# mmurooka/SMPLpp

Measured on AMD Instinct MI355X. Metric: SMPL FK evals/s + IK iters/s, batch 1024 frames, 1/2/4/8 MI355X, higher is better.
Workload: dtype f32 (exact operands: every fp32 value as three bf16 pieces = fp32's 24 bits on the bf16 matrix pipe, fp32 accumulate; fp32 VALU skinning)

## Files before the change

smplpp_amd/csrc/common.h:

```cpp
#pragma once

#include <hip/hip_runtime.h>

#include <cstdint>
#include <cstdio>
#include <cstring>
#include <memory>
#include <string>
#include <utility>
#include <vector>

#include "layout.h"

namespace smplpp_hip
{
__host__ __device__ inline int64_t bcol(int64_t v, int x)
{
  return (v / VG) * (3 * VG) + x * VG + (v % VG);
}

__host__ __device__ inline uint16_t bf16_rn_bits(float x)
{
  uint32_t u;
  memcpy(&u, &x, 4);
// ... 163 lines not shown
  int64_t VGPn = 0;
  smplpp_hip::DevPtr<uint8_t> B2h;
  float sB = 1.0f, sG = 1.0f;
  smplpp_hip::DevPtr<int> range_flag;
  smplpp_hip::DevPtr<uint8_t> B3e;
  char form = 'e';
  char form_ik = 'h';
  smplpp_hip::DevPtr<uint8_t> wIdx;
  smplpp_hip::DevPtr<float> wVal;
  smplpp_hip::DevPtr<float> wSum;
  smplpp_hip::DevPtr<float> J0;
  smplpp_hip::DevPtr<float> JS;
  smplpp_hip::DevPtr<float> JSp;
  smplpp_hip::DevPtr<int32_t> parent;
  smplpp_hip::DevPtr<int32_t> lvl;
  int nlev = 0;
  bool chain_fast = false;
  smplpp_hip::DevPtr<int32_t> faces;
  smplpp_hip::DevPtr<int32_t> adjOff;
  smplpp_hip::DevPtr<int32_t> adjFace;
  int madj = smplpp_hip::MAXADJ;
  smplpp_hip::DevPtr<uint16_t> faceRing;
  smplpp_hip::DevPtr<uint8_t> faceMap;
  smplpp_hip::DevPtr<int32_t> anc;
  smplpp_hip::DevPtr<float> Wdense;
  smplpp_hip::DevPtr<float> Pvm;
  smplpp_hip::DevPtr<float> Svm;
  std::vector<int32_t> h_parent, h_faces, h_adjOff, h_adjFace;
  bool profiling = false;
  std::vector<hipEvent_t> prof_events;
  smplpp_hip::Workspace ws;
  smplpp_hip::Arena arena;
  smplpp_hip::StatePtr<smplpp_hip::VjpState> vjp;
  smplpp_hip::StatePtr<smplpp_hip::NormalsVjpState> nvjp;
  char pd_form = 0;
  smplpp_hip::StatePtr<smplpp_hip::PointDistState> pd;
  smplpp_hip::StatePtr<smplpp_hip::MeshPointDistState> mpd;
  smplpp_hip::StatePtr<smplpp_hip::WindingState> wn;
  smplpp_hip::StatePtr<smplpp_hip::SelfPenState> sp;
  int dr_inline = -1;
  smplpp_hip::StatePtr<smplpp_hip::DepthRasterState> dr;
  smplpp_hip::StatePtr<smplpp_hip::SilhouetteState> sil;
  int vo_frames = 0;
  smplpp_hip::StatePtr<smplpp_hip::VertexOffsetsState> vo;
  ~smplpp_model();
};
// ... 1 lines not shown
```

smplpp_amd/csrc/ik.hip:

```cpp
#include "ik_types.h"
#include "ik_eval.h"
#include "ik_solve.h"
#include "ik_proj.h"
#include "vposer_state.h"

#include <algorithm>
#include <chrono>
#include <cstdlib>
#include <type_traits>

using namespace smplpp_hip;

struct smplpp_ik
{
  smplpp_model * m = nullptr;
  smplpp_vposer * vp = nullptr;
  int64_t n = 0, K = 0;
  int64_t frame_base = 0;
  int theta_dim = TD75;
  TaskArrays ta{};
  float *theta = nullptr, *beta = nullptr, *theta25 = nullptr, *vjac = nullptr;
  float *verts = nullptr, *rest = nullptr, *joints = nullptr, *poserot = nullptr, *pts = nullptr;
  double *e = nullptr, *J = nullptr, *Jl = nullptr, *e2 = nullptr, *xout = nullptr;
  int *skip = nullptr, *status = nullptr, *sticky = nullptr, *list_cnt = nullptr, *list_f = nullptr;
// ... 1 lines not shown
  int32_t * roles = nullptr;
  float * list_d = nullptr;
  std::vector<DevPtr<void>> owned;
  bool have_eval = false;
  int64_t last_D = 0;
  hipStream_t side = nullptr;
  hipEvent_t ev_fork = nullptr, ev_join = nullptr;
  bool phi_locked = false;
  bool side_pending = false;
  int * dbg_buf = nullptr;
  unsigned * sig = nullptr;
  unsigned tick_fork = 0, tick_join = 0, tick_done = 0;
  bool use_flags = false;
  double last_enqueue_us = 0.0;
  bool latent_split = false;
  bool latent_split_default = false;
  bool exact = false;
  StatePtr<VPoserJxWork> jxw;
  bool jac_ahead = false;
  bool dbg_sync = false, overlap_ok = true;
  int dbg_stop = 0;
  int64_t scan_blocks = 1536;
  int scan_form = -1;
  float * vbuf[2] = {nullptr, nullptr};
  int vcur = 0;
  Arena arena;
  ~smplpp_ik()
  {
    (void)hipSetDevice(m->device);
    if(side) (void)hipStreamSynchronize(side);
    if(ev_fork) (void)hipEventDestroy(ev_fork);
    if(ev_join) (void)hipEventDestroy(ev_join);
    if(side) (void)hipStreamDestroy(side);
  }
};

enum Fill { AS_ALLOCATED, ZERO_BYTES, VALUE, DEFAULT_NORMAL };

template<class T>
static hipError_t dalloc(smplpp_ik * s, T *& p, size_t count, Fill fill, float v = 0.0f)
{
  DevPtr<T> d;
  hipError_t e = dev_alloc(d, count);
  p = d.get();
  if(e != hipSuccess) return e;
  s->owned.emplace_back(std::move(d));
// ... 69 lines not shown
  if(m->V > 65535) return fail(SMPLPP_ERR_INVALID, "smplpp_ik_create: at most 65535 vertices are supported (ring tables hold 16-bit ids)");
  if(!m->faceRing || !m->faceMap || !m->anc) return fail(SMPLPP_ERR_INVALID, "smplpp_ik_create: the model carries no ring tables");
  std::vector<int32_t> roles;
  if(const char * why = eval_roles(m->h_parent, EVAL_NT, roles)) return fail(SMPLPP_ERR_INVALID, why);
  if(K > PROJ_MAXK) return fail(SMPLPP_ERR_INVALID, "smplpp_ik_create: at most 48 tasks per frame are supported");
  if(TD75 + 2 * K + NB > MAXD)
    return fail(SMPLPP_ERR_INVALID, "smplpp_ik_create: too many tasks for the in-LDS solver (75 + 2K + 10 must be <= 181)");
  HIP_TRY(hipSetDevice(m->device));
  std::unique_ptr<smplpp_ik> s(new smplpp_ik());
  s->m = m;
  s->vp = vposer;
  s->n = n;
  s->K = K;
  s->theta_dim = vposer ? TD44 : TD75;
  {
    const char * e;
    s->dbg_sync = getenv("SMPLPP_DEBUG_SYNC") != nullptr;
    if((e = getenv("SMPLPP_IK_DBG_STOP"))) s->dbg_stop = atoi(e);
    if((e = getenv("SMPLPP_IK_OVERLAP"))) s->overlap_ok = e[0] != '0';
    if(s->dbg_sync) s->overlap_ok = false;
    s->scan_blocks = default_scan_blocks(n, K, m->F);
    if((e = getenv("SMPLPP_SCAN_BLOCKS"))) s->scan_blocks = atoll(e);
    if((e = getenv("SMPLPP_SCAN_FORM"))) s->scan_form = atoi(e);
    s->latent_split = vposer != nullptr && n <= 128 && s->dbg_stop == 0;
    if((e = getenv("SMPLPP_IK_LATENT_SPLIT"))) s->latent_split = vposer != nullptr && e[0] != '0' && s->dbg_stop == 0;
  }
  const size_t nk = (size_t)n * K;
  const size_t Dmax = TD75 + 2 * K + NB;
  const size_t nV3 = (size_t)n * m->V * 3;
  smplpp_ik * const p = s.get();
  HIP_TRY(dalloc(p, p->ta.face, nk, ZERO_BYTES));
  HIP_TRY(dalloc(p, p->ta.vw, nk * 3, VALUE, 1.0f / 3.0f));
  HIP_TRY(dalloc(p, p->ta.tang, nk * 6, VALUE, 0.0f));
  HIP_TRY(dalloc(p, p->ta.tpos, nk * 3, VALUE, 0.0f));
  HIP_TRY(dalloc(p, p->ta.tnrm, nk * 3, DEFAULT_NORMAL));
  HIP_TRY(dalloc(p, p->ta.posw, nk, VALUE, 1.0f));
  HIP_TRY(dalloc(p, p->ta.nrmw, nk, VALUE, 1.0f));
  HIP_TRY(dalloc(p, p->ta.philim, nk, VALUE, 0.04f));
  HIP_TRY(dalloc(p, p->ta.noff, nk, VALUE, 0.0f));
  HIP_TRY(dalloc(p, p->ta.apos, nk * 3, AS_ALLOCATED));
  HIP_TRY(dalloc(p, p->ta.anrm, nk * 3, AS_ALLOCATED));
  HIP_TRY(dalloc(p, p->ta.hint, nk, AS_ALLOCATED));
  HIP_TRY(dalloc(p, p->ta.roww, nk * 2, AS_ALLOCATED));
  HIP_TRY(dalloc(p, p->theta, (size_t)n * p->theta_dim, ZERO_BYTES));
  HIP_TRY(dalloc(p, p->beta, (size_t)n * NB, ZERO_BYTES));
  HIP_TRY(dalloc(p, p->theta25, (size_t)n * 75, ZERO_BYTES));
// ... 336 lines not shown
                                               solve_form<false, 3>()};
  return forms;
}

static int ik_enqueue_solve(smplpp_ik * s, const SolveCall & c)
{
  {
    TraceRange tr_solve("solve IK");
    const SolveForm * f = solve_forms();
    while(f->dual_only != c.p.dual_only || f->ntr != c.p.ntr) f++;
    f->launch(s, c);
  }
  HIP_TRY(hipGetLastError());
  return SMPLPP_OK;
}

template<int KPR, int NBT>
static void scan_launch(smplpp_ik * s, int chunks, const float * qpts, const float * hint, hipStream_t pst)
{
  proj_scan_kernel<KPR, NBT><<<dim3((unsigned)(s->n * chunks)), dim3(256), 0, pst>>>(view_of(s->m), s->ta, s->verts, qpts, hint, s->m->F, (int)s->K, chunks,
                                                                                    s->skip, s->list_cnt, s->list_d, s->list_f, s->dbg_stop);
}

static int ik_enqueue_reproject(smplpp_ik * s, const SidePlan & sp, int it, const SeqHook * last, hipStream_t st)
{
  smplpp_model * m = s->m;
  const int K = (int)s->K;
  const bool dbg = s->dbg_sync, beside = sp.beside;
  TraceRange tr_proj("project point");
  const float * qpts = beside ? s->ta.apos : s->pts;
  hipStream_t pst = st;
  if(beside)
  {
    if(s->use_flags)
      HIP_TRY(hipStreamWaitValue32(s->side, s->sig, s->tick_fork, hipStreamWaitValueGte, 0xffffffffu));
    else
      HIP_TRY(hipStreamWaitEvent(s->side, s->ev_fork, 0));
    pst = s->side;
  }
  const ScanPlan sc = scan_plan(s->n, K, m->F, s->scan_blocks, s->scan_form);
  const float * hint = beside ? s->ta.hint : nullptr;
  if(sc.nbt3) scan_launch<0, 3>(s, sc.chunks, qpts, hint, pst);
  else if(sc.kpr == 0) scan_launch<0, CP_BATCH>(s, sc.chunks, qpts, hint, pst);
  else if(sc.kpr == 2) scan_launch<2, CP_BATCH>(s, sc.chunks, qpts, hint, pst);
  else scan_launch<4, CP_BATCH>(s, sc.chunks, qpts, hint, pst);
  HIP_TRY(hipGetLastError());
  int *& dbg_buf = s->dbg_buf;
  if(dbg && !dbg_buf) HIP_TRY(dalloc(s, dbg_buf, 8, AS_ALLOCATED));
  if(dbg) HIP_TRY(hipMemsetAsync(dbg_buf, 0, sizeof(int) * 8, st));
  const int fsplit = frame_split(s->n, K);
  if(sp.go) s->tick_join++;
  hipExtLaunchKernelGGL(proj_finish_kernel, dim3((unsigned)(s->n * fsplit)), dim3(256), 0, pst, nullptr,
                        (beside && !s->use_flags) ? s->ev_join : nullptr, 0,
                        view_of(m), s->ta, (const float *)s->verts, qpts, m->F, K, (const int *)s->skip, s->list_cnt, s->list_d,
                        s->list_f, dbg ? dbg_buf : (int *)nullptr, fsplit, sp.join_flag ? s->sig + 32 : (unsigned *)nullptr,
                        sp.join_flag ? s->sig + 48 : (unsigned *)nullptr, s->tick_join, last ? last->next_tpos : (const float *)nullptr,
                        last ? last->next_valid : (const uint8_t *)nullptr, last ? last->shared : 0);
  HIP_TRY(hipGetLastError());
  if(sp.ahead)
  {
    HIP_TRY(hipStreamWaitValue32(s->side, s->sig + 64, s->tick_done, hipStreamWaitValueGte, 0xffffffffu));
    int rc = vposer_forward_device(s->vp, s->n, s->theta + 6, TD44, nullptr, 75, s->vjac, s->side, s->frame_base, false, s->sig + 32,
                                   s->sig + 48, s->tick_join);
    if(rc) return rc;
    s->jac_ahead = true;
  }
  if(beside) s->side_pending = true;
  if(dbg)
  {
    int h[8];
    HIP_TRY(hipMemcpy(h, dbg_buf, sizeof(h), hipMemcpyDeviceToHost));
    fprintf(stderr, "[smplpp dbg] it %d: project lists: tasks %d, empty %d, overflow %d, nan %d, max cnt %d\n", it, h[0], h[1], h[2], h[3], h[4]);
  }
  return SMPLPP_OK;
}

static int ik_iterate_enqueue(smplpp_ik * s, int iters, int enable_qp, int optimize_beta_from, int64_t min_valid, hipStream_t st,
                              const SeqHook * hook = nullptr, bool more_follows = false)
{
  int rc = SMPLPP_OK;
  const int K = (int)s->K;
  static PerDeviceOnce once_solve[SOLVE_FORMS];
  for(int i = 0; i < SOLVE_FORMS; i++) HIP_TRY(lds_opt_in(once_solve[i], s->m->device, solve_forms()[i].kfn, (int)SOLVE_LDS_MAX));
  if(s->use_flags && (s->tick_fork > 0x7fff0000u || s->tick_join > 0x7fff0000u || s->tick_done > 0x7fff0000u))
  {
    HIP_TRY(hipStreamSynchronize(st));
    HIP_TRY(hipStreamSynchronize(s->side));
    HIP_TRY(hipMemset(s->sig, 0, sizeof(unsigned) * 128));
    s->tick_fork = s->tick_join = s->tick_done = 0;
  }
  auto dbg_sync = [&](int it, const char * tag) -> int {
    if(!s->dbg_sync) return SMPLPP_OK;
    fprintf(stderr, "[smplpp dbg] it %d: %s ...\n", it, tag);
    HIP_TRY(hipStreamSynchronize(st));
    fprintf(stderr, "[smplpp dbg] it %d: %s done\n", it, tag);
// ... 174 lines not shown
```

smplpp_amd/csrc/ik_plan.h:

```cpp
#pragma once

#include <algorithm>
#include <cstddef>
#include <vector>

#include "layout.h"

namespace smplpp_hip
{
constexpr int TD75 = SMPLPP_THETA_DIM;
constexpr int TD44 = SMPLPP_LATENT_POSE_DIM;
constexpr int IK_MAXK = 48;
constexpr size_t SOLVE_LDS_MAX = 160 * 1024 - 1536;
constexpr int MAXD = TD75 + 2 * IK_MAXK + NB;

struct IterFlags
{
  int opt_beta, phi_live;
};
inline IterFlags iter_flags(int optimize_beta_from, int it)
{
  const int on = (optimize_beta_from >= 0 && it >= optimize_beta_from) ? 1 : 0;
  return {on, optimize_beta_from >= 0 ? on : 1};
}
// ... 37 lines not shown

inline int64_t default_scan_blocks(int64_t n, int64_t K, int64_t F)
{
  if(n >= 512 && K <= 8 && (F + 767) / 768 <= 32) return n * ((F + 767) / 768);
  return (n >= 256 && n < 512) ? 2 * n : 1536;
}

struct ScanPlan
{
  int chunks;
  int kpr;
  bool nbt3;
};
inline ScanPlan scan_plan(int64_t n, int K, int64_t F, int64_t scan_blocks, int scan_form)
{
  int chunks = (int)(scan_blocks / n);
  chunks = chunks < 1 ? 1 : (chunks > 32 ? 32 : chunks);
  const bool small_chunk = (F + chunks - 1) / chunks <= 3 * 256;
  const bool many = scan_form < 0 ? (n >= 512 && small_chunk) : scan_form == 0;
  const int kpr = (K > 8 || many) ? 0 : (K <= 4 ? 2 : 4);
  return {chunks, kpr, kpr == 0 && small_chunk};
}

inline int frame_split(int64_t n, int K)
{
  const int split = n < 256 ? (int)(256 / n) : 1;
  return std::max(1, std::min(split, K));
}

struct SidePlan
{
  bool beside;
  bool go;
  bool ahead;
  bool join_flag;
};
inline SidePlan side_plan(bool overlap_ok, bool phi_free, bool use_flags, bool latent_split, bool opt_beta, bool another_follows)
{
  SidePlan p;
  p.beside = overlap_ok && !phi_free;
  p.go = p.beside && use_flags;
  p.ahead = latent_split && p.go && !opt_beta && another_follows;
  p.join_flag = p.go && !p.ahead;
  return p;
}

// ... 25 lines not shown
```

smplpp_amd/csrc/ik_proj.h:

```cpp
#pragma once
#include "ik_types.h"

namespace smplpp_hip
{
constexpr int PROJ_LIST = 512;
constexpr int PROJ_MAXK = IK_MAXK;

typedef float f32x2 __attribute__((ext_vector_type(2)));

template<int KPR, int NBT = CP_BATCH>
__global__ __launch_bounds__(256) void proj_scan_kernel(ModelView mv, TaskArrays ta, const float * __restrict__ verts_all,
                                                         const float * __restrict__ pts, const float * __restrict__ hint, int64_t F,
                                                         int K, int chunks, const int * __restrict__ skip, int * __restrict__ list_cnt,
                                                         float * __restrict__ list_d, int * __restrict__ list_f, int dbg_stop)
{
  const int64_t f = blockIdx.x / chunks;
  const int chunk = blockIdx.x % chunks;
  if(skip[f]) return;
  const float * verts = verts_all + f * mv.V * 3;
  __shared__ float sp[PROJ_MAXK + 1][3];
  __shared__ float sreach[PROJ_MAXK + 1];
  __shared__ float sbound[PROJ_MAXK + 1];
  const int64_t tb = f * K;
  if((int)threadIdx.x < K)
  {
    const int k = threadIdx.x;
    const float * p = pts + (tb + k) * 3;
    sp[k][0] = p[0];
    sp[k][1] = p[1];
    sp[k][2] = p[2];
    float d;
    if(hint)
      d = hint[tb + k];
    else
    {
      float c[3];
      d = tri_sqdist_dev(verts, mv.faces, ta.face[tb + k], p, c);
    }
    sreach[k] = (d == d) ? sqrtf(d) : INFINITY;
    sbound[k] = (d == d) ? d * 1.00001f + 2e-12f : INFINITY;
  }
  else if((int)threadIdx.x == K)
  {
    sp[K][0] = sp[K][1] = sp[K][2] = 1e18f;
    sreach[K] = 0.0f;
    sbound[K] = 0.0f;
  }
  __syncthreads();
  if(dbg_stop == 10) return;
  f32x2 qx[KPR > 0 ? KPR : 1], qy[KPR > 0 ? KPR : 1], qz[KPR > 0 ? KPR : 1], qs[KPR > 0 ? KPR : 1];
  if(KPR > 0)
  {
#pragma unroll
    for(int q = 0; q < KPR; q++)
    {
      const int k0 = (2 * q < K) ? 2 * q : K, k1 = (2 * q + 1 < K) ? 2 * q + 1 : K;
      qx[q] = f32x2{sp[k0][0], sp[k1][0]};
      qy[q] = f32x2{sp[k0][1], sp[k1][1]};
      qz[q] = f32x2{sp[k0][2], sp[k1][2]};
      qs[q] = f32x2{sreach[k0], sreach[k1]};
    }
  }
  const int64_t per = (F + chunks - 1) / chunks;
  const int64_t f_lo = chunk * per, f_hi = (f_lo + per < F) ? f_lo + per : F;
  for(int64_t base = f_lo + threadIdx.x; base < f_hi; base += (int64_t)blockDim.x * NBT)
  {
    TriBatchT<NBT> t;
    load_tri_batch(verts, mv.faces, f_hi, base, blockDim.x, t);
    if(dbg_stop == 11) { if(t.v[0][0] == 12345.678f) list_cnt[0] = 1; continue; }
#pragma unroll
    for(int b = 0; b < NBT; b++)
    {
      if(!t.valid[b]) continue;
      const int64_t face = base + (int64_t)b * blockDim.x;
      const float * a = t.v[b];
      const float g[3] = {(a[0] + a[3] + a[6]) * (1.0f / 3.0f), (a[1] + a[4] + a[7]) * (1.0f / 3.0f), (a[2] + a[5] + a[8]) * (1.0f / 3.0f)};
      float r2 = 0.0f;
#pragma unroll
      for(int c = 0; c < 3; c++)
      {
        const float dx = a[c * 3] - g[0], dy = a[c * 3 + 1] - g[1], dz = a[c * 3 + 2] - g[2];
        r2 = fmaxf(r2, dx * dx + dy * dy + dz * dz);
      }
      const float r = __builtin_amdgcn_sqrtf(r2) * 1.000001f;
      uint64_t hit = 0;
      if(KPR > 0)
      {
#pragma unroll
        for(int q = 0; q < KPR; q++)
        {
          const f32x2 dx = qx[q] - g[0], dy = qy[q] - g[1], dz = qz[q] - g[2];
          const f32x2 d0 = dx * dx + dy * dy + dz * dz;
          const f32x2 reach = (qs[q] + r) * 1.00001f + 2e-6f;
          const f32x2 rr = reach * reach;
          hit |= (d0.x <= rr.x) ? (1ull << (2 * q)) : 0ull;
          hit |= (d0.y <= rr.y) ? (1ull << (2 * q + 1)) : 0ull;
        }
      }
      else
      {
        for(int k = 0; k < K; k++)
        {
          const float d0 = (sp[k][0] - g[0]) * (sp[k][0] - g[0]) + (sp[k][1] - g[1]) * (sp[k][1] - g[1]) + (sp[k][2] - g[2]) * (sp[k][2] - g[2]);
          const float reach = (sreach[k] + r) * 1.00001f + 2e-6f;
          hit |= (d0 <= reach * reach) ? (1ull << k) : 0ull;
        }
      }
      while(hit)
      {
        const int k = __builtin_ctzll(hit);
        hit &= hit - 1;
        const float d = tri_sqdist_vals(a[0], a[1], a[2], a[3], a[4], a[5], a[6], a[7], a[8], sp[k][0], sp[k][1], sp[k][2]).x;
        if(!(d <= sbound[k])) continue;
        const int slot = atomicAdd(&list_cnt[tb + k], 1);
        if(slot < PROJ_LIST)
        {
          list_d[(tb + k) * PROJ_LIST + slot] = d;
          list_f[(tb + k) * PROJ_LIST + slot] = (int)face;
        }
      }
    }
  }
}

__device__ __forceinline__ void proj_finish_body(const ModelView & mv, const TaskArrays & ta, const float * __restrict__ verts_all,
                                                 const float * __restrict__ pts, int64_t F, int K,
                                                 const int * __restrict__ skip, int * __restrict__ list_cnt,
                                                 const float * __restrict__ list_d, const int * __restrict__ list_f,
                                                 int * __restrict__ dbg, int tsplit)
{
  const int64_t f = blockIdx.x / tsplit;
  const int part = (int)(blockIdx.x % tsplit), per_part = (K + tsplit - 1) / tsplit;
  const int k_begin = part * per_part, k_end = (k_begin + per_part < K) ? k_begin + per_part : K;
  const int64_t tb = f * K;
  if(skip[f]) return;
  const float * verts = verts_all + f * mv.V * 3;
  __shared__ int s_face[PROJ_MAXK];
  __shared__ int s_slow[PROJ_MAXK];
  for(int k0 = k_begin; k0 < k_end; k0 += 8)
  {
    const int k = k0 + (int)threadIdx.x / 32, l = (int)threadIdx.x % 32;
    const bool live = k < k_end;
    const int cnt = live ? list_cnt[tb + k] : 0;
// ... 117 lines not shown
```

smplpp_amd/csrc/ik_types.h:

```cpp
#pragma once
#include "ik_plan.h"
#include "mesh_device.h"
#include "staging.h"
#include "trace.h"
#include "signal.h"

#include <hip/hip_ext.h>

struct smplpp_vposer;

namespace smplpp_hip
{
int fk_device(smplpp_model * m, int64_t n, const float * beta, const float * theta, float * verts, float * joints,
              float * xforms44, float * rest, float * poserot, hipStream_t st, int range_slot, int * range_word = nullptr,
              char form_override = 0);
int vposer_forward_device(smplpp_vposer * v, int64_t n, const float * z, int64_t z_stride, float * out, int64_t out_stride,
                          float * jac, hipStream_t st, int64_t frame_base, bool value_like_jac = false, unsigned * sig_flag = nullptr,
                          unsigned * sig_counter = nullptr, unsigned sig_tick = 0u);

constexpr int NQ = TD75 + NB;

struct TaskArrays
{
  int32_t * face;
// ... 12 lines not shown
  float * roww;
};

struct ModelView
{
  const int32_t * faces;
  const int32_t * adjOff;
  const int32_t * adjFace;
  const int32_t * parent;
  const uint8_t * wIdx;
  const float * wVal;
  const float * wSum;
  const float * Pvm;
  const float * Svm;
  const float * JS;
  const uint16_t * faceRing;
  const uint8_t * faceMap;
  const int32_t * anc;
  int nlev;
  int64_t V;
  int maxw;
};

__device__ inline void lds_barrier()
{
  asm volatile("s_waitcnt lgkmcnt(0)\n\ts_barrier" ::: "memory");
}

#ifndef SMPLPP_EVAL_NT
#define SMPLPP_EVAL_NT 768
#endif
constexpr int EVAL_NT = SMPLPP_EVAL_NT;
#ifdef SMPLPP_EVAL_STAMPS
__device__ unsigned long long g_eval_stamps[64 * 16];
#define EVAL_STAMP(i) do { if(tid == 0 && blockIdx.x < 64) g_eval_stamps[blockIdx.x * 16 + (i)] = __builtin_readcyclecounter(); } while(0)
#else
#define EVAL_STAMP(i) do {} while(0)
#endif
#ifdef SMPLPP_SOLVE_STAMPS
__device__ unsigned long long g_solve_stamps[64 * 16];
#define SOLVE_STAMP(i) do { if(threadIdx.x == 0 && blockIdx.x < 64) g_solve_stamps[blockIdx.x * 16 + (i)] = __builtin_amdgcn_s_memrealtime(); } while(0)
#else
#define SOLVE_STAMP(i) do {} while(0)
#endif
}
```

smplpp_amd/csrc/layout.h:

```cpp
#pragma once

#include <cstdint>

#include "../../include/smplpp_hip.h"

namespace smplpp_hip
{
constexpr int NJ = SMPLPP_JOINT_NUM;
constexpr int NB = SMPLPP_SHAPE_BASIS_DIM;
constexpr int NP = SMPLPP_POSE_BASIS_DIM;

constexpr int KP = 220;
constexpr int K_BETA = NP;
constexpr int K_ONE = NP + NB;
constexpr int CT_LEV = 12;
constexpr int CT_OFF = 52;
constexpr int CT_P_R = 0, CT_P_J = SMPLPP_JOINT_NUM * 9, CT_P_ZERO = CT_P_J + SMPLPP_JOINT_NUM * 3, CT_P_SIZE = CT_P_ZERO + 4;
constexpr int TREE_DMAX = 12;
constexpr int TREE_ANC = 0, TREE_LVL = SMPLPP_JOINT_NUM, TREE_LVLJ = TREE_LVL + TREE_DMAX + 1, TREE_SIZE = TREE_LVLJ + SMPLPP_JOINT_NUM;
constexpr int RANGE_DEVICE = 0, RANGE_HOST = 1, RANGE_INTERNAL = 2, RANGE_SLOTS = 4;
constexpr int MAXADJ = 12;
constexpr int MAXADJ_WIDE = 16;
constexpr int MAXRING = 3 * (MAXADJ + 1) + 1;
constexpr int VG = 32;

constexpr int BB_KS = 14;
constexpr int BB_A_BYTES = 6 * 1024;
constexpr int BB_B_BYTES = 18 * 1024;
constexpr int BB_KSTEP_BYTES = BB_A_BYTES + BB_B_BYTES;

constexpr int EB_KS = 14;
constexpr int EB_IMG = 20 * 1024;
constexpr int EB_TAB_OFF = 18 * 1024;

constexpr int HB_KS = 14;
constexpr int HB_SLOTS = 15;
constexpr int HB_A_BYTES = 4 * 1024;
constexpr int HB_IMG = 12 * 1024;
constexpr int HB_G_BYTES = 72 * 1024;
constexpr int HB_CW_OFF = 8 * 1024;
constexpr int HB_PERM_OFF = HB_CW_OFF + 256;
constexpr int HB_FLAGS_OFF = HB_CW_OFF + 512;
constexpr float HB_SA = 64.0f;
constexpr float HB_SW = 16384.0f;
}
```

smplpp_amd/csrc/model.hip:

```cpp
#include "common.h"
#include "model_tables.h"

#include <cstdlib>
#include <tuple>

namespace smplpp_hip
{
typedef _Float16 f16x8h __attribute__((ext_vector_type(8)));
static thread_local std::string g_last_error;

void set_error(const std::string & msg)
{
  g_last_error = msg;
}

int fail(int code, const std::string & msg)
{
  g_last_error = msg;
  return code;
}

int hip_fail(hipError_t e, const char * what, const char * file, int line)
{
  char buf[512];
// ... 270 lines not shown
  m->F = F;
  m->VGn = (V + VG - 1) / VG;
  m->ldB = m->VGn * 3 * VG;
  m->VGPn = (V + 63) / 64;

  const SkinWeights sw = skin_weights(W, V);
  m->maxw = sw.maxw;
  read_env(*m);
  auto uses = [&](char f) { return m->form == f || m->form_ik == f; };
  VertexGroups hgroups;
  if(uses('h'))
  {
    const HScales hs = h_scales(P, S, vt, V);
    if(hs.refusal) return fail(SMPLPP_ERR_INVALID, hs.refusal);
    m->sB = hs.sB;
    m->sG = hs.sG;
    hgroups = h_vertex_groups(W, V);
  }
  const JointLevels levels = joint_levels(parent);
  const ChainTables chain = chain_tables(parent, levels);
  const std::vector<int32_t> anc = ik_tree_tables(parent, levels);
  Adjacency adj = adjacency(faces1, F, V);
  const RingTables ring = ik_ring_tables(adj.faces.data(), adj.adjOff.data(), adj.adjFace.data(), F, V);
  m->nlev = levels.nlev;
  m->chain_fast = chain.chain_fast;
  m->madj = ring.madj;
  m->h_parent = parent;
  m->h_faces = std::move(adj.faces);
  m->h_adjOff = std::move(adj.adjOff);
  m->h_adjFace = std::move(adj.adjFace);

  HIP_TRY(upload(m->Pvm, P, (size_t)V * 3 * NP));
  HIP_TRY(upload(m->Svm, S, (size_t)V * 3 * NB));
  DevPtr<float> dT, dJreg;
  HIP_TRY(upload(dT, vt, (size_t)V * 3));
  HIP_TRY(upload(dJreg, Jreg, (size_t)NJ * V));
  HIP_TRY(dev_alloc(m->Bm, (size_t)KP * m->ldB));
  HIP_TRY(dev_alloc(m->J0, NJ * 3));
  HIP_TRY(dev_alloc(m->JS, NJ * 3 * NB));
  relayout_basis_kernel<<<dim3((unsigned)((m->ldB + 255) / 256)), dim3(256)>>>(m->Pvm.get(), m->Svm.get(), dT.get(), m->Bm.get(), V, m->ldB);
  fold_regressor_kernel<<<dim3(NJ * 3 * (NB + 1)), dim3(256)>>>(dJreg.get(), m->Svm.get(), dT.get(), m->J0.get(), m->JS.get(), V);
  HIP_TRY(dev_alloc(m->JSp, NJ * 3 * 12));
  pack_regressor_rows_kernel<<<dim3(1), dim3(NJ * 3)>>>(m->J0.get(), m->JS.get(), m->JSp.get());
  if(uses('b'))
  {
    HIP_TRY(dev_alloc(m->B3, (size_t)m->VGPn * BB_KS * BB_B_BYTES));
// ... 30 lines not shown
    const int64_t cnt = m->VGPn * (HB_KS * 6 * 64 + 4 * 64 + 64);
    relayout_basis_f16x2_kernel<<<dim3((unsigned)((cnt + 255) / 256)), dim3(256)>>>(m->Bm.get(), m->ldB, m->Wdense.get(), m->wSum.get(), V,
                                                                                 m->VGPn, m->sB, m->sG, m->B2h.get(), dPerm.get(), dFlags.get());
    HIP_TRY(hipGetLastError());
    HIP_TRY(hipDeviceSynchronize());
  }
  if(!uses('v')) m->Bm.reset();

  HIP_TRY(upload(m->parent, parent.data(), parent.size()));
  {
    const int zero[RANGE_SLOTS] = {};
    HIP_TRY(upload(m->range_flag, zero, RANGE_SLOTS));
  }
  HIP_TRY(upload(m->lvl, chain.lvl.data(), chain.lvl.size()));
  HIP_TRY(upload(m->faces, m->h_faces.data(), m->h_faces.size()));
  HIP_TRY(upload(m->adjOff, m->h_adjOff.data(), m->h_adjOff.size()));
  HIP_TRY(upload(m->adjFace, m->h_adjFace.data(), m->h_adjFace.size()));
  HIP_TRY(upload(m->anc, anc.data(), anc.size()));
  if(!ring.faceRing.empty())
  {
    HIP_TRY(upload(m->faceRing, ring.faceRing.data(), ring.faceRing.size()));
    HIP_TRY(upload(m->faceMap, ring.faceMap.data(), ring.faceMap.size()));
  }
  *out = m.release();
  return SMPLPP_OK;
}

extern "C" int smplpp_model_info(const smplpp_model * m, int64_t * V, int64_t * F, int * wpv, int * device)
{
  if(!m) return fail(SMPLPP_ERR_INVALID, "smplpp_model_info: null model");
  if(V) *V = m->V;
  if(F) *F = m->F;
  if(wpv) *wpv = m->maxw;
  if(device) *device = m->device;
  return SMPLPP_OK;
}

extern "C" int smplpp_adjacent_faces(const smplpp_model * m, int64_t vertex, int64_t cap, int64_t * faces, float * weights,
                                     int64_t * count)
{
  if(!m || !count) return fail(SMPLPP_ERR_INVALID, "smplpp_adjacent_faces: null argument");
  if(vertex < 0 || vertex >= m->V) return fail(SMPLPP_ERR_INVALID, "smplpp_adjacent_faces: vertex out of range");
  int32_t b = m->h_adjOff[vertex], e = m->h_adjOff[vertex + 1];
  *count = e - b;
  float sum = 0.0f;
  for(int32_t q = b; q < e; q++) sum += 1.0f;
// ... 8 lines not shown
```

smplpp_amd/csrc/model_tables.h:

```cpp
#pragma once

#include <algorithm>
#include <cmath>
#include <cstdint>
#include <utility>
#include <vector>

#include "layout.h"

namespace smplpp_hip
{
inline const char * check_tree(const int64_t * kintree, std::vector<int32_t> & parent)
{
  parent.assign(NJ, -1);
  for(int i = 1; i < NJ; i++)
  {
    if(kintree[i] < 0 || kintree[i] >= i) return "Cannot set kinematic tree: parent(i) must precede i";
    parent[i] = (int32_t)kintree[i];
  }
  return nullptr;
}
inline const char * check_faces(const int32_t * faces1, int64_t F, int64_t V)
{
  for(int64_t i = 0; i < F * 3; i++)
// ... 255 lines not shown
    {
      const int32_t u = faces[f * 3 + i], b0 = adjOff[u];
      const int cnt = std::min<int>(adjOff[u + 1] - b0, MADJ_);
      for(int a = 0; a < cnt; a++)
        for(int cc = 0; cc < 3; cc++)
        {
          const int32_t v = faces[(int64_t)adjFace[b0 + a] * 3 + cc];
          int slot = -1;
          for(int q = 0; q < nr; q++)
            if(rg[1 + q] == (uint16_t)v) slot = q;
          if(slot < 0 && nr < MRING_)
          {
            slot = nr;
            rg[1 + nr++] = (uint16_t)v;
          }
          mp[(i * MADJ_ + a) * 3 + cc] = (uint8_t)(slot < 0 ? 0 : slot);
        }
    }
    rg[0] = (uint16_t)nr;
  }
  return t;
}

inline std::pair<char, char> choose_forms(const char * env, int maxw, int64_t VGPn)
{
  const char e = env ? env[0] : 0;
  char forms[2] = {'e', 'h'};
  if(e == 'e' || e == 'h' || e == 'b' || e == 'v') forms[0] = forms[1] = e;
  for(char & f : forms)
  {
    if(f == 'h' && VGPn * HB_SLOTS * HB_IMG > 0x7fffff00LL) f = 'v';
    if(f == 'e' && VGPn * EB_KS * EB_IMG > 0x7fffff00LL) f = 'v';
    if(f == 'b' && VGPn * BB_KS * BB_B_BYTES > 0x7fffff00LL) f = 'v';
    if(f == 'e' && maxw > 4) f = 'b';
    if(f == 'b' && maxw > 8) f = 'v';
  }
  return {forms[0], forms[1]};
}
}
```

Baseline: 15.28 million.

## Cull projection face scan with per-frame cluster bounding boxes

Precomputes face clusters built by BFS over adjacency, along with per-cluster vertex tile lists. A new cull kernel builds each cluster's AABB from the current posed vertices, tests it against every query's reach sphere, then compacts the surviving clusters with a prefix sum. Only faces in those clusters are tested, and only against the queries that survived, instead of brute-force scanning all faces. The cost is an extra AABB pass over every vertex plus binary-search indexing and gathered vertex loads for each surviving triangle.

```diff
diff --git a/smplpp_amd/csrc/common.h b/smplpp_amd/csrc/common.h
--- a/smplpp_amd/csrc/common.h
+++ b/smplpp_amd/csrc/common.h
@@ -209,6 +209,10 @@
   int madj = smplpp_hip::MAXADJ;
   smplpp_hip::DevPtr<uint16_t> faceRing;
   smplpp_hip::DevPtr<uint8_t> faceMap;
+  int sc_ncl = 0;
+  int sc_octets = 0;
+  smplpp_hip::DevPtr<int32_t> clOff, clTri, faceCl;
+  smplpp_hip::DevPtr<uint16_t> clTileV;
   smplpp_hip::DevPtr<int32_t> anc;
   smplpp_hip::DevPtr<float> Wdense;
   smplpp_hip::DevPtr<float> Pvm;
diff --git a/smplpp_amd/csrc/ik.hip b/smplpp_amd/csrc/ik.hip
--- a/smplpp_amd/csrc/ik.hip
+++ b/smplpp_amd/csrc/ik.hip
@@ -47,6 +47,7 @@
   int dbg_stop = 0;
   int64_t scan_blocks = 1536;
   int scan_form = -1;
+  int scan_cull = 1;
   float * vbuf[2] = {nullptr, nullptr};
   int vcur = 0;
   Arena arena;
@@ -162,6 +163,7 @@
     s->scan_blocks = default_scan_blocks(n, K, m->F);
     if((e = getenv("SMPLPP_SCAN_BLOCKS"))) s->scan_blocks = atoll(e);
     if((e = getenv("SMPLPP_SCAN_FORM"))) s->scan_form = atoi(e);
+    if((e = getenv("SMPLPP_SCAN_CULL"))) s->scan_cull = atoi(e);
     s->latent_split = vposer != nullptr && n <= 128 && s->dbg_stop == 0;
     if((e = getenv("SMPLPP_IK_LATENT_SPLIT"))) s->latent_split = vposer != nullptr && e[0] != '0' && s->dbg_stop == 0;
   }
@@ -544,6 +546,19 @@
                                                                                     s->skip, s->list_cnt, s->list_d, s->list_f, s->dbg_stop);
 }
 
+static ClusterView clusters_of(const smplpp_model * m)
+{
+  return {m->clOff.get(), m->clTri.get(), m->clTileV.get(), m->sc_octets, m->faceCl.get(), m->sc_ncl};
+}
+constexpr int CULL_NBT = 3;
+static int cull_launch(smplpp_ik * s, const CullPlan & cp, const float * qpts, const float * hint, int * dbg, hipStream_t pst)
+{
+  proj_cull_kernel<CULL_NBT><<<dim3((unsigned)(s->n * cp.groups)), dim3(CULL_NT), 0, pst>>>(view_of(s->m), clusters_of(s->m), s->ta, s->verts, qpts, hint,
+                                                                                                s->m->F, (int)s->K, cp.groups, s->skip, s->list_cnt,
+                                                                                                s->list_d, s->list_f, dbg);
+  return SMPLPP_OK;
+}
+
 static int ik_enqueue_reproject(smplpp_ik * s, const SidePlan & sp, int it, const SeqHook * last, hipStream_t st)
 {
   smplpp_model * m = s->m;
@@ -562,14 +577,19 @@
   }
   const ScanPlan sc = scan_plan(s->n, K, m->F, s->scan_blocks, s->scan_form);
   const float * hint = beside ? s->ta.hint : nullptr;
-  if(sc.nbt3) scan_launch<0, 3>(s, sc.chunks, qpts, hint, pst);
+  const CullPlan cp = cull_plan(s->n, K, m->F, m->sc_ncl, s->scan_cull);
+  int *& dbg_buf = s->dbg_buf;
+  if(dbg && !dbg_buf) HIP_TRY(dalloc(s, dbg_buf, 8, AS_ALLOCATED));
+  if(dbg) HIP_TRY(hipMemsetAsync(dbg_buf, 0, sizeof(int) * 8, st));
+  if(cp.use)
+  {
+    if(int rc = cull_launch(s, cp, qpts, hint, dbg ? dbg_buf : nullptr, pst)) return rc;
+  }
+  else if(sc.nbt3) scan_launch<0, 3>(s, sc.chunks, qpts, hint, pst);
   else if(sc.kpr == 0) scan_launch<0, CP_BATCH>(s, sc.chunks, qpts, hint, pst);
   else if(sc.kpr == 2) scan_launch<2, CP_BATCH>(s, sc.chunks, qpts, hint, pst);
   else scan_launch<4, CP_BATCH>(s, sc.chunks, qpts, hint, pst);
   HIP_TRY(hipGetLastError());
-  int *& dbg_buf = s->dbg_buf;
-  if(dbg && !dbg_buf) HIP_TRY(dalloc(s, dbg_buf, 8, AS_ALLOCATED));
-  if(dbg) HIP_TRY(hipMemsetAsync(dbg_buf, 0, sizeof(int) * 8, st));
   const int fsplit = frame_split(s->n, K);
   if(sp.go) s->tick_join++;
   hipExtLaunchKernelGGL(proj_finish_kernel, dim3((unsigned)(s->n * fsplit)), dim3(256), 0, pst, nullptr,
@@ -593,6 +613,7 @@
     int h[8];
     HIP_TRY(hipMemcpy(h, dbg_buf, sizeof(h), hipMemcpyDeviceToHost));
     fprintf(stderr, "[smplpp dbg] it %d: project lists: tasks %d, empty %d, overflow %d, nan %d, max cnt %d\n", it, h[0], h[1], h[2], h[3], h[4]);
+    if(cp.use) fprintf(stderr, "[smplpp dbg] it %d: project cull: clusters tested %d, surviving %d\n", it, h[5], h[6]);
   }
   return SMPLPP_OK;
 }
diff --git a/smplpp_amd/csrc/ik_plan.h b/smplpp_amd/csrc/ik_plan.h
--- a/smplpp_amd/csrc/ik_plan.h
+++ b/smplpp_amd/csrc/ik_plan.h
@@ -83,6 +83,20 @@
   return {chunks, kpr, kpr == 0 && small_chunk};
 }
 
+struct CullPlan
+{
+  bool use;
+  int groups;
+};
+inline CullPlan cull_plan(int64_t n, int K, int64_t F, int ncl, int cull_mode)
+{
+  CullPlan p{false, 1};
+  if(cull_mode <= 0 || n <= 0 || K <= 0 || F <= 0 || ncl <= 0 || ncl > SC_MAXCL) return p;
+  p.use = true;
+  p.groups = (int)std::max<int64_t>(1, std::min<int64_t>(std::min<int64_t>(8, ncl), 256 / n));
+  return p;
+}
+
 inline int frame_split(int64_t n, int K)
 {
   const int split = n < 256 ? (int)(256 / n) : 1;
diff --git a/smplpp_amd/csrc/ik_proj.h b/smplpp_amd/csrc/ik_proj.h
--- a/smplpp_amd/csrc/ik_proj.h
+++ b/smplpp_amd/csrc/ik_proj.h
@@ -8,20 +8,24 @@
 
 typedef float f32x2 __attribute__((ext_vector_type(2)));
 
-template<int KPR, int NBT = CP_BATCH>
-__global__ __launch_bounds__(256) void proj_scan_kernel(ModelView mv, TaskArrays ta, const float * __restrict__ verts_all,
-                                                         const float * __restrict__ pts, const float * __restrict__ hint, int64_t F,
-                                                         int K, int chunks, const int * __restrict__ skip, int * __restrict__ list_cnt,
-                                                         float * __restrict__ list_d, int * __restrict__ list_f, int dbg_stop)
-{
-  const int64_t f = blockIdx.x / chunks;
-  const int chunk = blockIdx.x % chunks;
-  if(skip[f]) return;
-  const float * verts = verts_all + f * mv.V * 3;
-  __shared__ float sp[PROJ_MAXK + 1][3];
-  __shared__ float sreach[PROJ_MAXK + 1];
-  __shared__ float sbound[PROJ_MAXK + 1];
-  const int64_t tb = f * K;
+struct ScanQueries
+{
+  float sp[PROJ_MAXK + 1][3];
+  float sreach[PROJ_MAXK + 1];
+  float sbound[PROJ_MAXK + 1];
+};
+template<int KPR>
+struct QueryRegs
+{
+  f32x2 qx[KPR > 0 ? KPR : 1], qy[KPR > 0 ? KPR : 1], qz[KPR > 0 ? KPR : 1], qs[KPR > 0 ? KPR : 1];
+};
+
+__device__ __forceinline__ void scan_load_queries(ScanQueries & sq, const ModelView & mv, const TaskArrays & ta, const float * __restrict__ verts,
+                                                  const float * __restrict__ pts, const float * __restrict__ hint, int64_t tb, int K)
+{
+  float (&sp)[PROJ_MAXK + 1][3] = sq.sp;
+  float (&sreach)[PROJ_MAXK + 1] = sq.sreach;
+  float (&sbound)[PROJ_MAXK + 1] = sq.sbound;
   if((int)threadIdx.x < K)
   {
     const int k = threadIdx.x;
@@ -46,21 +50,101 @@
     sreach[K] = 0.0f;
     sbound[K] = 0.0f;
   }
+}
+
+template<int KPR>
+__device__ __forceinline__ void scan_query_regs(const ScanQueries & sq, int K, QueryRegs<KPR> & qr)
+{
+  if(KPR > 0)
+  {
+#pragma unroll
+    for(int q = 0; q < KPR; q++)
+    {
+      const int k0 = (2 * q < K) ? 2 * q : K, k1 = (2 * q + 1 < K) ? 2 * q + 1 : K;
+      qr.qx[q] = f32x2{sq.sp[k0][0], sq.sp[k1][0]};
+      qr.qy[q] = f32x2{sq.sp[k0][1], sq.sp[k1][1]};
+      qr.qz[q] = f32x2{sq.sp[k0][2], sq.sp[k1][2]};
+      qr.qs[q] = f32x2{sq.sreach[k0], sq.sreach[k1]};
+    }
+  }
+}
+
+template<int KPR, bool MASKED = false>
+__device__ __forceinline__ void scan_test_face(const float * a, int64_t face, int K, const ScanQueries & sq, const QueryRegs<KPR> & qr,
+                                               int64_t tb, int * __restrict__ list_cnt, float * __restrict__ list_d, int * __restrict__ list_f,
+                                               uint64_t allow = 0)
+{
+  const float (&sp)[PROJ_MAXK + 1][3] = sq.sp;
+  const float (&sreach)[PROJ_MAXK + 1] = sq.sreach;
+  const float (&sbound)[PROJ_MAXK + 1] = sq.sbound;
+  const f32x2 * qx = qr.qx, * qy = qr.qy, * qz = qr.qz, * qs = qr.qs;
+  const float g[3] = {(a[0] + a[3] + a[6]) * (1.0f / 3.0f), (a[1] + a[4] + a[7]) * (1.0f / 3.0f), (a[2] + a[5] + a[8]) * (1.0f / 3.0f)};
+  float r2 = 0.0f;
+#pragma unroll
+  for(int c = 0; c < 3; c++)
+  {
+    const float dx = a[c * 3] - g[0], dy = a[c * 3 + 1] - g[1], dz = a[c * 3 + 2] - g[2];
+    r2 = fmaxf(r2, dx * dx + dy * dy + dz * dz);
+  }
+  const float r = __builtin_amdgcn_sqrtf(r2) * 1.000001f;
+  uint64_t hit = 0;
+  if(KPR > 0)
+  {
+#pragma unroll
+    for(int q = 0; q < KPR; q++)
+    {
+      const f32x2 dx = qx[q] - g[0], dy = qy[q] - g[1], dz = qz[q] - g[2];
+      const f32x2 d0 = dx * dx + dy * dy + dz * dz;
+      const f32x2 reach = (qs[q] + r) * 1.00001f + 2e-6f;
+      const f32x2 rr = reach * reach;
+      hit |= (d0.x <= rr.x) ? (1ull << (2 * q)) : 0ull;
+      hit |= (d0.y <= rr.y) ? (1ull << (2 * q + 1)) : 0ull;
+    }
+  }
+  else
+  {
+    auto one = [&](int k) {
+      const float d0 = (sp[k][0] - g[0]) * (sp[k][0] - g[0]) + (sp[k][1] - g[1]) * (sp[k][1] - g[1]) + (sp[k][2] - g[2]) * (sp[k][2] - g[2]);
+      const float reach = (sreach[k] + r) * 1.00001f + 2e-6f;
+      hit |= (d0 <= reach * reach) ? (1ull << k) : 0ull;
+    };
+    if(MASKED)
+      for(uint64_t m = allow; m; m &= m - 1) one(__builtin_ctzll(m));
+    else
+      for(int k = 0; k < K; k++) one(k);
+  }
+  while(hit)
+  {
+    const int k = __builtin_ctzll(hit);
+    hit &= hit - 1;
+    const float d = tri_sqdist_vals(a[0], a[1], a[2], a[3], a[4], a[5], a[6], a[7], a[8], sp[k][0], sp[k][1], sp[k][2]).x;
+    if(!(d <= sbound[k])) continue;
+    const int slot = atomicAdd(&list_cnt[tb + k], 1);
+    if(slot < PROJ_LIST)
+    {
+      list_d[(tb + k) * PROJ_LIST + slot] = d;
+      list_f[(tb + k) * PROJ_LIST + slot] = (int)face;
+    }
+  }
+}
+
+template<int KPR, int NBT = CP_BATCH>
+__global__ __launch_bounds__(256) void proj_scan_kernel(ModelView mv, TaskArrays ta, const float * __restrict__ verts_all,
+                                                         const float * __restrict__ pts, const float * __restrict__ hint, int64_t F,
+                                                         int K, int chunks, const int * __restrict__ skip, int * __restrict__ list_cnt,
+                                                         float * __restrict__ list_d, int * __restrict__ list_f, int dbg_stop)
+{
+  const int64_t f = blockIdx.x / chunks;
+  const int chunk = blockIdx.x % chunks;
+  if(skip[f]) return;
+  const float * verts = verts_all + f * mv.V * 3;
+  __shared__ ScanQueries sq;
+  const int64_t tb = f * K;
+  scan_load_queries(sq, mv, ta, verts, pts, hint, tb, K);
   __syncthreads();
   if(dbg_stop == 10) return;
-  f32x2 qx[KPR > 0 ? KPR : 1], qy[KPR > 0 ? KPR : 1], qz[KPR > 0 ? KPR : 1], qs[KPR > 0 ? KPR : 1];
-  if(KPR > 0)
-  {
-#pragma unroll
-    for(int q = 0; q < KPR; q++)
-    {
-      const int k0 = (2 * q < K) ? 2 * q : K, k1 = (2 * q + 1 < K) ? 2 * q + 1 : K;
-      qx[q] = f32x2{sp[k0][0], sp[k1][0]};
-      qy[q] = f32x2{sp[k0][1], sp[k1][1]};
-      qz[q] = f32x2{sp[k0][2], sp[k1][2]};
-      qs[q] = f32x2{sreach[k0], sreach[k1]};
-    }
-  }
+  QueryRegs<KPR> qr;
+  scan_query_regs<KPR>(sq, K, qr);
   const int64_t per = (F + chunks - 1) / chunks;
   const int64_t f_lo = chunk * per, f_hi = (f_lo + per < F) ? f_lo + per : F;
   for(int64_t base = f_lo + threadIdx.x; base < f_hi; base += (int64_t)blockDim.x * NBT)
@@ -72,53 +156,198 @@
     for(int b = 0; b < NBT; b++)
     {
       if(!t.valid[b]) continue;
-      const int64_t face = base + (int64_t)b * blockDim.x;
-      const float * a = t.v[b];
-      const float g[3] = {(a[0] + a[3] + a[6]) * (1.0f / 3.0f), (a[1] + a[4] + a[7]) * (1.0f / 3.0f), (a[2] + a[5] + a[8]) * (1.0f / 3.0f)};
-      float r2 = 0.0f;
-#pragma unroll
-      for(int c = 0; c < 3; c++)
+      scan_test_face<KPR>(t.v[b], base + (int64_t)b * blockDim.x, K, sq, qr, tb, list_cnt, list_d, list_f);
+    }
+  }
+}
+
+constexpr int CULL_NT = 256;
+template<int NBT>
+__global__ __launch_bounds__(CULL_NT) void proj_cull_kernel(ModelView mv, ClusterView cv, TaskArrays ta, const float * __restrict__ verts_all,
+                                                             const float * __restrict__ pts, const float * __restrict__ hint, int64_t F,
+                                                             int K, int groups, const int * __restrict__ skip, int * __restrict__ list_cnt,
+                                                             float * __restrict__ list_d, int * __restrict__ list_f, int * __restrict__ dbg)
+{
+  const int64_t f = blockIdx.x / groups;
+  const int part = blockIdx.x % groups;
+  if(skip[f]) return;
+  const int tid = threadIdx.x;
+  const int V = (int)mv.V;
+  const float * verts = verts_all + f * mv.V * 3;
+  __shared__ float s_tile[SC_TILE * 3];
+  __shared__ ScanQueries sq;
+  __shared__ int s_owncl[PROJ_MAXK + 1];
+  __shared__ int s_start[SC_MAXCL];
+  __shared__ uint64_t s_mask[SC_MAXCL];
+  __shared__ int s_pref[SC_MAXCL + 1];
+  __shared__ int s_nsurv;
+  const int64_t tb = f * K;
+  const int ncl = cv.ncl;
+  scan_load_queries(sq, mv, ta, verts, pts, hint, tb, K);
+  if(tid < K)
+  {
+    const int own = ta.face[tb + tid];
+    s_owncl[tid] = (own >= 0 && (int64_t)own < F) ? cv.faceCl[own] : -1;
+  }
+  if(tid == 0) s_nsurv = 0;
+  static_assert(SC_MAXCL <= CULL_NT, "one cluster per thread");
+  const int c = part + groups * tid;
+  const bool mine = c < ncl;
+  const int passes = (V + SC_TILE - 1) / SC_TILE;
+  const uint4 * octets = reinterpret_cast<const uint4 *>(cv.clTileV);
+  float lo[3] = {INFINITY, INFINITY, INFINITY}, hi[3] = {-INFINITY, -INFINITY, -INFINITY};
+  const int o_n = mine ? cv.octets : 0;
+  const int first = mine ? cv.clOff[c] : 0, cnt = mine ? cv.clOff[c + 1] - first : 0;
+  for(int p = 0; p < passes; p++)
+  {
+    const int v_lo = p * SC_TILE, nt3 = ((V - v_lo < SC_TILE) ? V - v_lo : SC_TILE) * 3;
+    const int o_lo = (c * passes + p) * cv.octets;
+    constexpr int OB = 8;
+    uint4 ids[OB];
+#pragma unroll
+    for(int q = 0; q < OB; q++) ids[q] = mine ? octets[o_lo + q] : make_uint4(~0u, ~0u, ~0u, ~0u);
+    if(p) __syncthreads();
+    {
+      const float * src = verts + v_lo * 3;
+      const int head = (int)((4 - ((reinterpret_cast<uintptr_t>(src) >> 2) & 3)) & 3);
+      const int nq = nt3 > head ? (nt3 - head) / 4 : 0;
+      const float4 * src4 = reinterpret_cast<const float4 *>(src + head);
+      constexpr int QPT = (SC_TILE * 3 / 4 + CULL_NT - 1) / CULL_NT;
+      float4 q4[QPT];
+#pragma unroll
+      for(int j = 0; j < QPT; j++)
+        if(tid + j * CULL_NT < nq) q4[j] = src4[tid + j * CULL_NT];
+#pragma unroll
+      for(int j = 0; j < QPT; j++)
+        if(tid + j * CULL_NT < nq)
+        {
+          float * dst = s_tile + head + 4 * (tid + j * CULL_NT);
+          dst[0] = q4[j].x;
+          dst[1] = q4[j].y;
+          dst[2] = q4[j].z;
+          dst[3] = q4[j].w;
+        }
+      if(tid < head && tid < nt3) s_tile[tid] = src[tid];
+      const int done = head + 4 * nq;
+      if(done >= head && done + tid < nt3 && tid < 4) s_tile[done + tid] = src[done + tid];
+    }
+    __syncthreads();
+    for(int o = 0; o < o_n; o += OB)
+    {
+      if(o)
+#pragma unroll
+        for(int q = 0; q < OB; q++) ids[q] = octets[o_lo + o + q];
+#pragma unroll
+      for(int q = 0; q < OB; q++)
       {
-        const float dx = a[c * 3] - g[0], dy = a[c * 3 + 1] - g[1], dz = a[c * 3 + 2] - g[2];
-        r2 = fmaxf(r2, dx * dx + dy * dy + dz * dz);
-      }
-      const float r = __builtin_amdgcn_sqrtf(r2) * 1.000001f;
-      uint64_t hit = 0;
-      if(KPR > 0)
-      {
-#pragma unroll
-        for(int q = 0; q < KPR; q++)
+        const unsigned w[4] = {ids[q].x, ids[q].y, ids[q].z, ids[q].w};
+#pragma unroll
+        for(int e = 0; e < 8; e++)
         {
-          const f32x2 dx = qx[q] - g[0], dy = qy[q] - g[1], dz = qz[q] - g[2];
-          const f32x2 d0 = dx * dx + dy * dy + dz * dz;
-          const f32x2 reach = (qs[q] + r) * 1.00001f + 2e-6f;
-          const f32x2 rr = reach * reach;
-          hit |= (d0.x <= rr.x) ? (1ull << (2 * q)) : 0ull;
-          hit |= (d0.y <= rr.y) ? (1ull << (2 * q + 1)) : 0ull;
+          const unsigned v = (w[e >> 1] >> (16 * (e & 1))) & 0xffffu;
+          if(v == SC_NOVERT) continue;
+          const float * x = s_tile + 3 * v;
+#pragma unroll
+          for(int d = 0; d < 3; d++)
+          {
+            lo[d] = fminf(lo[d], x[d]);
+            hi[d] = fmaxf(hi[d], x[d]);
+          }
         }
       }
-      else
+    }
+  }
+  int tested = 0, kept = 0;
+  if(mine)
+  {
+    uint64_t mask = 0;
+    for(int k = 0; k < K; k++)
+    {
+      const float dx = fmaxf(fmaxf(lo[0] - sq.sp[k][0], sq.sp[k][0] - hi[0]), 0.0f);
+      const float dy = fmaxf(fmaxf(lo[1] - sq.sp[k][1], sq.sp[k][1] - hi[1]), 0.0f);
+      const float dz = fmaxf(fmaxf(lo[2] - sq.sp[k][2], sq.sp[k][2] - hi[2]), 0.0f);
+      const float l2 = dx * dx + dy * dy + dz * dz;
+      const float R = sq.sreach[k] * 1.0001f + 1e-5f;
+      if(!(l2 > R * R) || s_owncl[k] == c) mask |= 1ull << k;
+    }
+    tested = 1;
+    if(mask && cnt > 0)
+    {
+      kept = 1;
+      const int slot = atomicAdd(&s_nsurv, 1);
+      s_start[slot] = first;
+      s_mask[slot] = mask;
+      s_pref[slot] = cnt;
+    }
+  }
+  if(dbg && tested)
+  {
+    atomicAdd(&dbg[5], tested);
+    atomicAdd(&dbg[6], kept);
+  }
+  __syncthreads();
+  const int ns = s_nsurv;
+  if(tid < 64)
+  {
+    const int per = (ns + 63) / 64;
+    int sum = 0;
+    for(int i = 0; i < per; i++)
+      if(tid * per + i < ns) sum += s_pref[tid * per + i];
+    int incl = sum;
+#pragma unroll
+    for(int o = 1; o < 64; o <<= 1)
+    {
+      const int up = __shfl_up(incl, o, 64);
+      if(tid >= o) incl += up;
+    }
+    int run = incl - sum;
+    for(int i = 0; i < per; i++)
+      if(tid * per + i < ns)
       {
-        for(int k = 0; k < K; k++)
-        {
-          const float d0 = (sp[k][0] - g[0]) * (sp[k][0] - g[0]) + (sp[k][1] - g[1]) * (sp[k][1] - g[1]) + (sp[k][2] - g[2]) * (sp[k][2] - g[2]);
-          const float reach = (sreach[k] + r) * 1.00001f + 2e-6f;
-          hit |= (d0 <= reach * reach) ? (1ull << k) : 0ull;
-        }
+        const int cnt = s_pref[tid * per + i];
+        s_pref[tid * per + i] = run;
+        run += cnt;
       }
-      while(hit)
+    if(tid == 63) s_pref[ns] = incl;
+  }
+  __syncthreads();
+  const int total = s_pref[ns];
+  const QueryRegs<0> qr{};
+  const int4 * tri = reinterpret_cast<const int4 *>(cv.clTri);
+  for(int base = tid; base < total; base += CULL_NT * NBT)
+  {
+    int4 id[NBT];
+    uint64_t allow[NBT];
+#pragma unroll
+    for(int b = 0; b < NBT; b++)
+    {
+      const int i = base + b * CULL_NT;
+      const int ii = i < total ? i : 0;
+      int s_lo = 0, s_hi = ns - 1;
+      while(s_lo < s_hi)
       {
-        const int k = __builtin_ctzll(hit);
-        hit &= hit - 1;
-        const float d = tri_sqdist_vals(a[0], a[1], a[2], a[3], a[4], a[5], a[6], a[7], a[8], sp[k][0], sp[k][1], sp[k][2]).x;
-        if(!(d <= sbound[k])) continue;
-        const int slot = atomicAdd(&list_cnt[tb + k], 1);
-        if(slot < PROJ_LIST)
-        {
-          list_d[(tb + k) * PROJ_LIST + slot] = d;
-          list_f[(tb + k) * PROJ_LIST + slot] = (int)face;
-        }
+        const int mid = (s_lo + s_hi + 1) >> 1;
+        if(s_pref[mid] <= ii) s_lo = mid;
+        else s_hi = mid - 1;
       }
+      id[b] = tri[s_start[s_lo] + (ii - s_pref[s_lo])];
+      allow[b] = i < total ? s_mask[s_lo] : 0ull;
+    }
+    float a[NBT][9];
+#pragma unroll
+    for(int b = 0; b < NBT; b++)
+    {
+      const int vi[3] = {id[b].x, id[b].y, id[b].z};
+#pragma unroll
+      for(int c = 0; c < 3; c++)
+#pragma unroll
+        for(int d = 0; d < 3; d++) a[b][c * 3 + d] = verts[3 * vi[c] + d];
+    }
+#pragma unroll
+    for(int b = 0; b < NBT; b++)
+    {
+      if(!allow[b]) continue;
+      scan_test_face<0, true>(a[b], id[b].w, K, sq, qr, tb, list_cnt, list_d, list_f, allow[b]);
     }
   }
 }
diff --git a/smplpp_amd/csrc/ik_types.h b/smplpp_amd/csrc/ik_types.h
--- a/smplpp_amd/csrc/ik_types.h
+++ b/smplpp_amd/csrc/ik_types.h
@@ -58,6 +58,16 @@
   int maxw;
 };
 
+struct ClusterView
+{
+  const int32_t * clOff;
+  const int32_t * clTri;
+  const uint16_t * clTileV;
+  int octets;
+  const int32_t * faceCl;
+  int ncl;
+};
+
 __device__ inline void lds_barrier()
 {
   asm volatile("s_waitcnt lgkmcnt(0)\n\ts_barrier" ::: "memory");
diff --git a/smplpp_amd/csrc/layout.h b/smplpp_amd/csrc/layout.h
--- a/smplpp_amd/csrc/layout.h
+++ b/smplpp_amd/csrc/layout.h
@@ -22,6 +22,8 @@
 constexpr int MAXADJ = 12;
 constexpr int MAXADJ_WIDE = 16;
 constexpr int MAXRING = 3 * (MAXADJ + 1) + 1;
+constexpr int SC_FACES = 64, SC_MAXCL = 256, SC_TILE = 3456;
+constexpr unsigned SC_NOVERT = 0xffffu;
 constexpr int VG = 32;
 
 constexpr int BB_KS = 14;
diff --git a/smplpp_amd/csrc/model.hip b/smplpp_amd/csrc/model.hip
--- a/smplpp_amd/csrc/model.hip
+++ b/smplpp_amd/csrc/model.hip
@@ -316,6 +316,7 @@
   const std::vector<int32_t> anc = ik_tree_tables(parent, levels);
   Adjacency adj = adjacency(faces1, F, V);
   const RingTables ring = ik_ring_tables(adj.faces.data(), adj.adjOff.data(), adj.adjFace.data(), F, V);
+  const ScanClusters clusters = scan_clusters(adj.faces.data(), adj.adjOff.data(), adj.adjFace.data(), F, V);
   m->nlev = levels.nlev;
   m->chain_fast = chain.chain_fast;
   m->madj = ring.madj;
@@ -392,6 +393,15 @@
     HIP_TRY(upload(m->faceRing, ring.faceRing.data(), ring.faceRing.size()));
     HIP_TRY(upload(m->faceMap, ring.faceMap.data(), ring.faceMap.size()));
   }
+  if(clusters.ncl > 0)
+  {
+    m->sc_ncl = clusters.ncl;
+    HIP_TRY(upload(m->clOff, clusters.clOff.data(), clusters.clOff.size()));
+    HIP_TRY(upload(m->clTri, clusters.clTri.data(), clusters.clTri.size()));
+    m->sc_octets = clusters.octets;
+    HIP_TRY(upload(m->clTileV, clusters.clTileV.data(), clusters.clTileV.size()));
+    HIP_TRY(upload(m->faceCl, clusters.faceCl.data(), clusters.faceCl.size()));
+  }
   *out = m.release();
   return SMPLPP_OK;
 }
diff --git a/smplpp_amd/csrc/model_tables.h b/smplpp_amd/csrc/model_tables.h
--- a/smplpp_amd/csrc/model_tables.h
+++ b/smplpp_amd/csrc/model_tables.h
@@ -301,6 +301,91 @@
   return t;
 }
 
+struct ScanClusters
+{
+  int ncl = 0;
+  std::vector<int32_t> clOff;
+  std::vector<int32_t> clTri;
+  std::vector<int32_t> clVOff;
+  std::vector<uint16_t> clVert;
+  int passes = 0;
+  int octets = 0;
+  std::vector<uint16_t> clTileV;
+  std::vector<int32_t> faceCl;
+};
+inline ScanClusters scan_clusters(const int32_t * faces, const int32_t * adjOff, const int32_t * adjFace, int64_t F, int64_t V)
+{
+  ScanClusters t;
+  if(F <= 0 || V <= 0 || V > 65535) return t;
+  int ncl = 0;
+  for(int64_t target = SC_FACES;; target *= 2)
+  {
+    t.faceCl.assign((size_t)F, -1);
+    ncl = 0;
+    std::vector<int32_t> queue;
+    for(int64_t seed = 0; seed < F; seed++)
+    {
+      if(t.faceCl[seed] >= 0) continue;
+      queue.assign(1, (int32_t)seed);
+      t.faceCl[seed] = ncl;
+      for(size_t head = 0; head < queue.size() && (int64_t)queue.size() < target; head++)
+        for(int i = 0; i < 3; i++)
+        {
+          const int32_t v = faces[(int64_t)queue[head] * 3 + i];
+          for(int32_t q = adjOff[v]; q < adjOff[v + 1] && (int64_t)queue.size() < target; q++)
+            if(t.faceCl[adjFace[q]] < 0)
+            {
+              t.faceCl[adjFace[q]] = ncl;
+              queue.push_back(adjFace[q]);
+            }
+        }
+      ncl++;
+    }
+    if(ncl <= SC_MAXCL) break;
+    if(target >= F) return ScanClusters();
+  }
+  t.ncl = ncl;
+  t.clOff.assign((size_t)ncl + 1, 0);
+  for(int64_t f = 0; f < F; f++) t.clOff[(size_t)t.faceCl[f] + 1]++;
+  for(int c = 0; c < ncl; c++) t.clOff[c + 1] += t.clOff[c];
+  t.clTri.resize((size_t)F * 4);
+  std::vector<int32_t> fill(t.clOff.begin(), t.clOff.end() - 1);
+  std::vector<std::vector<uint16_t>> vs((size_t)ncl);
+  for(int64_t f = 0; f < F; f++)
+  {
+    const int c = t.faceCl[f];
+    int32_t * q = t.clTri.data() + (size_t)fill[c]++ * 4;
+    for(int i = 0; i < 3; i++)
+    {
+      q[i] = faces[f * 3 + i];
+      vs[c].push_back((uint16_t)faces[f * 3 + i]);
+    }
+    q[3] = (int32_t)f;
+  }
+  t.clVOff.assign((size_t)ncl + 1, 0);
+  for(int c = 0; c < ncl; c++)
+  {
+    std::sort(vs[c].begin(), vs[c].end());
+    vs[c].erase(std::unique(vs[c].begin(), vs[c].end()), vs[c].end());
+    t.clVOff[c + 1] = t.clVOff[c] + (int32_t)vs[c].size();
+    t.clVert.insert(t.clVert.end(), vs[c].begin(), vs[c].end());
+  }
+  t.passes = (int)((V + SC_TILE - 1) / SC_TILE);
+  std::vector<std::vector<uint16_t>> rel((size_t)ncl * t.passes);
+  size_t most = 1;
+  for(int c = 0; c < ncl; c++)
+    for(uint16_t v : vs[c])
+    {
+      auto & r = rel[(size_t)c * t.passes + v / SC_TILE];
+      r.push_back((uint16_t)(v % SC_TILE));
+      most = std::max(most, r.size());
+    }
+  t.octets = (int)((most + 63) / 64 * 8);
+  t.clTileV.assign((size_t)ncl * t.passes * t.octets * 8, (uint16_t)SC_NOVERT);
+  for(size_t s = 0; s < rel.size(); s++) std::copy(rel[s].begin(), rel[s].end(), t.clTileV.begin() + s * t.octets * 8);
+  return t;
+}
+
 inline std::pair<char, char> choose_forms(const char * env, int maxw, int64_t VGPn)
 {
   const char e = env ? env[0] : 0;
```

New measurement: 15.20 million. Within noise of the previous version (-0.5%).
